# tinganchen/AlignQ

Measured on AMD Instinct MI355X. Metric: images/sec (train step, CDF+ADMM) ResNet-20 8-bit, higher is better.
Workload: dtype f32; 1 GPU; resnet20 CIFAR-shape 3x32x32, 8W/8A CDF+ADMM full train step (cdf_alignment_admm/resnet-20-cifar-10), batch 128/GPU, HIP-graph replay, batch-norm folded into the site kernels, channels-last tensors, all Conv2d_Q convolutions on alignq_conv*_nhwc (exact-product bf16 MFMA); global_batch=128, parallelism=dp1

## Files before the change

### alignq_amd/csrc/conv_kernels.hip

```cpp
#include <hip/hip_runtime.h>
#include <stdint.h>
#include <stdlib.h>

#include "../../include/alignq.h"
#include "site_internal.h"
#include "store_forms.h"
#include "wgrad_reduce_body.h"

namespace {

using namespace alignq_wgr;

typedef __bf16 bf16x8 __attribute__((ext_vector_type(8)));
typedef __bf16 bf16x4 __attribute__((ext_vector_type(4)));
typedef float f32x4 __attribute__((ext_vector_type(4)));
typedef short s16x4 __attribute__((ext_vector_type(4)));

#ifdef ALIGNQ_STAMPS
__device__ unsigned long long g_conv_stamps[64];
__device__ unsigned long long g_conv_blk[2][4096];
#define STAMP(on, i)                                                          \
  do {                                                                        \
    if ((on) && threadIdx.x == 0) g_conv_stamps[i] = wall_clock64();          \
  } while (0)
#define BSTAMP(which)                                                                          \
  do {                                                                                         \
    if (threadIdx.x == 0 && blockIdx.x < 4096) g_conv_blk[which][blockIdx.x] = wall_clock64(); \
  } while (0)
#else
#define STAMP(on, i) do { } while (0)
#define BSTAMP(which) do { } while (0)
#endif

__device__ __forceinline__ s16x4 tr_read(const __bf16* p) {
  return __builtin_amdgcn_ds_read_tr16_b64_v4i16((__attribute__((address_space(3))) s16x4*)(p));
}
__device__ __forceinline__ bf16x8 join8(s16x4 a, s16x4 b) {
  typedef short s16x8 __attribute__((ext_vector_type(8)));
  s16x8 v = {a[0], a[1], a[2], a[3], b[0], b[1], b[2], b[3]};
  return __builtin_bit_cast(bf16x8, v);
}


template <int xb>
__device__ __forceinline__ f32x4 fetch_act4(const float* __restrict__ x, int64_t off) {
  if constexpr (xb == 0) return *reinterpret_cast<const f32x4*>(x + off);
  if constexpr (xb == 2) {
    const s16x4 b = *reinterpret_cast<const s16x4*>(reinterpret_cast<const short*>(x) + off);
    return (f32x4){(float)b[0], (float)b[1], (float)b[2], (float)b[3]};
  }
  const char4 b = *reinterpret_cast<const char4*>(reinterpret_cast<const signed char*>(x) + off);
  return (f32x4){(float)b.x, (float)b.y, (float)b.z, (float)b.w};
}

struct BnLazy {
  const float* z;
  const float* ab;
  const float* save;
  const float* ktot;
  const float* part = nullptr;
  int n_tiles = 0, tile_f = 0;
  double inv_n = 1.0;
  float* dgamma = nullptr;
  float* dbeta = nullptr;
};

template <int C>
__device__ __forceinline__ void bn_totals_lds(const BnLazy& t, float* __restrict__ kt, bool publish) {
  static_assert(256 % C == 0, "thread -> (channel, group)");
  __shared__ double red[256][2];
  constexpr int G = 256 / C;
  const int tid = threadIdx.x;
  const int cp = C < t.tile_f ? C : t.tile_f;
  const int cyc = C / cp, cnt = t.n_tiles / cyc;
  const int c = tid % C, grp = tid / C;
  const int e = c % cp, t_first = c / cp;
  double s0 = 0, s1 = 0;
  constexpr int U = 16;
  for (int i0 = grp; i0 < cnt; i0 += G * U) {
    float2 v[U];
#pragma unroll
    for (int u = 0; u < U; u++) {
      const int i = i0 + u * G;
      const int ic = i < cnt ? i : cnt - 1;
      v[u] = *reinterpret_cast<const float2*>(t.part + ((int64_t)(ic * cyc + t_first) * cp + e) * 2);
    }
#pragma unroll
    for (int u = 0; u < U; u++) {
      if (i0 + u * G < cnt) { s0 += v[u].x; s1 += v[u].y; }
    }
  }
  red[tid][0] = s0;
  red[tid][1] = s1;
  __syncthreads();
  if (tid < C) {
    double t0 = 0, t1 = 0;
#pragma unroll
    for (int g = 0; g < G; g++) { t0 += red[g * C + tid][0]; t1 += red[g * C + tid][1]; }
    kt[tid] = (float)(t0 * t.inv_n);
    kt[C + tid] = (float)(t1 * t.inv_n);
    if (publish) {
      if (t.dbeta) t.dbeta[tid] = (float)t0;
      if (t.dgamma) t.dgamma[tid] = (float)t1;
    }
  }
  __syncthreads();
}

__device__ __forceinline__ float4 bn_lazy4(const float4& g, const float4& z, const float4& a, const float4& m, const float4& is,
                                           const float4& k0, const float4& k1) {
  float4 o;
  o.x = a.x * (g.x - k0.x - (z.x - m.x) * is.x * k1.x);
  o.y = a.y * (g.y - k0.y - (z.y - m.y) * is.y * k1.y);
  o.z = a.z * (g.z - k0.z - (z.z - m.z) * is.z * k1.z);
  o.w = a.w * (g.w - k0.w - (z.w - m.w) * is.w * k1.w);
  return o;
}

template <int C> constexpr int conv_cp() { return C == 16 ? 16 : (C == 32 ? 48 : C + 8); }
template <int C, int WD, int PT>
struct ConvLds {
  static constexpr int kBf16 = 3 * ((PT / WD) + 2) * (WD + 2) * conv_cp<C>();
};

template <int C, int WD, int PT, bool DGRAD, int XB = 0, bool IMG = false>
__device__ __forceinline__ void conv3x3_body(const float* __restrict__ x, const float* __restrict__ w,
                                             float* __restrict__ y, int H, int total_rows, float nlev, __bf16* lds,
                                             int block, const float* __restrict__ add,
                                             float* __restrict__ bn_part = nullptr, int n_wg = 0,
                                             BnLazy lazy = BnLazy{nullptr, nullptr, nullptr, nullptr}, float xlev = 1.0f) {
  static_assert(XB == 0 || !DGRAD, "the data gradient reads fp32 dy");
  constexpr int xb = XB;
  constexpr int TR = PT / WD;
  constexpr int NS = (9 * C + 31) / 32;
  constexpr int NCG = C / 16;
  constexpr int NPP = 4 / NCG;
  constexpr int NG = PT / 16;
  constexpr int LW = WD + 2;
  constexpr int CP = conv_cp<C>();
  constexpr int LROWS = TR + 2;
  constexpr int ARR = LROWS * LW * CP;
  static_assert(3 * ARR == ConvLds<C, WD, PT>::kBf16, "LDS size");
  __bf16* Xhi = lds;
  __bf16* Xmi = lds + ARR;
  __bf16* Xlo = lds + 2 * ARR;

  const int tid = threadIdx.x, lane = tid & 63, wv = tid >> 6;
  const int row0 = block * TR;
  const int img_lo = (row0 / H) * H, img_hi = img_lo + H;
  [[maybe_unused]] constexpr int SB = DGRAD ? 8 : 0;
  STAMP(block == 0, SB + 0);
  const int cog = wv % NCG, pp = wv / NCG;
  const int m = lane & 15, q = lane >> 4;
  bf16x8 ab[NS];
  {
    constexpr int C4 = C / 4;
    constexpr int N4 = LROWS * LW * C4;
    constexpr int NIT = (N4 + 255) / 256;
    float4 v[NIT];
#pragma unroll
    for (int it = 0; it < NIT; it++) {
      const int i = tid + 256 * it;
      const int c4 = i % C4, col = (i / C4) % LW, lr = i / (C4 * LW);
      const int grow = row0 + lr - 1;
      const bool ok = i < N4 && col >= 1 && col <= WD && grow >= img_lo && grow < img_hi && grow < total_rows;
      const int64_t off = ok ? ((int64_t)grow * WD + (col - 1)) * C + 4 * c4 : 0;
      const f32x4 ld = fetch_act4<XB>(x, off);
      v[it] = ok ? make_float4(ld[0], ld[1], ld[2], ld[3]) : make_float4(0.f, 0.f, 0.f, 0.f);
    }
    STAMP(block == 0, SB + 1);
    if (DGRAD && lazy.z) {
      float4 zz[NIT];
#pragma unroll
      for (int it = 0; it < NIT; it++) {
        const int i = tid + 256 * it;
        const int c4 = i % C4, col = (i / C4) % LW, lr = i / (C4 * LW);
        const int grow = row0 + lr - 1;
        const bool ok = i < N4 && col >= 1 && col <= WD && grow >= img_lo && grow < img_hi && grow < total_rows;
        zz[it] = *reinterpret_cast<const float4*>(lazy.z + (ok ? ((int64_t)grow * WD + (col - 1)) * C + 4 * c4 : 0));
      }
      const int c4t = tid % C4;
      const float4 a4 = *reinterpret_cast<const float4*>(lazy.ab + 4 * c4t);
      const float4 m4 = *reinterpret_cast<const float4*>(lazy.save + 4 * c4t);
      const float4 i4 = *reinterpret_cast<const float4*>(lazy.save + C + 4 * c4t);
      float4 k0, k1;
      if (lazy.part) {
        __shared__ __attribute__((aligned(16))) float kt[2 * C];
        bn_totals_lds<C>(lazy, kt, block == 0);
        k0 = *reinterpret_cast<const float4*>(kt + 4 * c4t);
        k1 = *reinterpret_cast<const float4*>(kt + C + 4 * c4t);
      } else {
        k0 = *reinterpret_cast<const float4*>(lazy.ktot + 4 * c4t);
        k1 = *reinterpret_cast<const float4*>(lazy.ktot + C + 4 * c4t);
      }
#pragma unroll
      for (int it = 0; it < NIT; it++) {
        const int i = tid + 256 * it;
        const int col = (i / C4) % LW, lr = i / (C4 * LW);
        const int grow = row0 + lr - 1;
        const bool ok = i < N4 && col >= 1 && col <= WD && grow >= img_lo && grow < img_hi && grow < total_rows;
        if (ok) v[it] = bn_lazy4(v[it], zz[it], a4, m4, i4, k0, k1);
      }
    }
#pragma unroll
    for (int it = 0; it < NIT; it++) {
      const int i = tid + 256 * it;
      if (i < N4) {
        const int c4 = i % C4, col = (i / C4) % LW, lr = i / (C4 * LW);
        bf16x4 h4, m4, l4;
        const float vv[4] = {v[it].x, v[it].y, v[it].z, v[it].w};
#pragma unroll
        for (int e = 0; e < 4; e++) {
          const __bf16 hi = (__bf16)vv[e];
          const float r1 = vv[e] - (float)hi;
          const __bf16 mi = (__bf16)r1;
          const float r2 = r1 - (float)mi;
          h4[e] = hi; m4[e] = mi; l4[e] = (__bf16)r2;
        }
        const int o = (lr * LW + col) * CP + 4 * c4;
        *reinterpret_cast<bf16x4*>(Xhi + o) = h4;
        *reinterpret_cast<bf16x4*>(Xmi + o) = m4;
        *reinterpret_cast<bf16x4*>(Xlo + o) = l4;
      }
    }
    STAMP(block == 0, SB + 2);
    if constexpr (IMG) {
      const bf16x8* __restrict__ wi = reinterpret_cast<const bf16x8*>(w) + (cog * NS) * 64 + lane;
#pragma unroll
      for (int s = 0; s < NS; s++) ab[s] = wi[s * 64];
    } else {
#pragma unroll
      for (int s = 0; s < NS; s++) {
        const int k0 = 32 * s + 8 * q;
        const bool live = k0 / C < 9;
        const int tap = live ? k0 / C : 8, c0 = k0 % C;
        float wr[8];
        if (!DGRAD) {
          const float* p = w + ((int64_t)(cog * 16 + m) * 9 + tap) * C + c0;
          const float4 a4 = *reinterpret_cast<const float4*>(p), b4 = *reinterpret_cast<const float4*>(p + 4);
          wr[0] = a4.x; wr[1] = a4.y; wr[2] = a4.z; wr[3] = a4.w; wr[4] = b4.x; wr[5] = b4.y; wr[6] = b4.z; wr[7] = b4.w;
        } else {
#pragma unroll
          for (int j = 0; j < 8; j++) wr[j] = w[((int64_t)(c0 + j) * 9 + (8 - tap)) * C + cog * 16 + m];
        }
#pragma unroll
        for (int j = 0; j < 8; j++) ab[s][j] = (__bf16)rintf((live ? wr[j] : 0.f) * nlev);
      }
    }
    STAMP(block == 0, SB + 3);
  }
  __syncthreads();
  constexpr int GW = NG / NPP;
  static_assert(NG % NPP == 0, "every wave takes the same number of pixel groups");
  int bo[GW];
  f32x4 acc[GW];
#pragma unroll
  for (int gi = 0; gi < GW; gi++) {
// ... 200 lines not shown
#pragma unroll
  for (int s = 0; s <= NS; s++) {
    if (s < NS) {
      const int k0 = 32 * s + 8 * q;
      const bool live = k0 / CIN < KS * KS;
      const int tap = live ? k0 / CIN : KS * KS - 1, c0 = k0 % CIN;
      const int to = (KS == 3 ? ((tap / KS) * LW + (tap % KS)) * CP : 0) + c0;
#pragma unroll
      for (int gi = 0; gi < GW; gi++) {
        const int o = bo[gi] + to;
        bh[s & 1][gi] = *reinterpret_cast<const bf16x8*>(Xhi + o);
        bm[s & 1][gi] = *reinterpret_cast<const bf16x8*>(Xmi + o);
        bl[s & 1][gi] = *reinterpret_cast<const bf16x8*>(Xlo + o);
        if ((KS * KS * CIN) % 32 != 0 && !live) {
#pragma unroll
          for (int j = 0; j < 8; j++) { bh[s & 1][gi][j] = (__bf16)0.f; bm[s & 1][gi][j] = (__bf16)0.f; bl[s & 1][gi][j] = (__bf16)0.f; }
        }
      }
    }
    __builtin_amdgcn_sched_barrier(0);
    if (s > 0) {
      const int u = s - 1;
#pragma unroll
      for (int gi = 0; gi < GW; gi++) {
        f32x4 a = acc[gi];
        a = __builtin_amdgcn_mfma_f32_16x16x32_bf16(ab[u], bl[u & 1][gi], a, 0, 0, 0);
        a = __builtin_amdgcn_mfma_f32_16x16x32_bf16(ab[u], bm[u & 1][gi], a, 0, 0, 0);
        acc[gi] = __builtin_amdgcn_mfma_f32_16x16x32_bf16(ab[u], bh[u & 1][gi], a, 0, 0, 0);
      }
    }
  }
  float bs[4] = {0.f, 0.f, 0.f, 0.f}, bq[4] = {0.f, 0.f, 0.f, 0.f};
#pragma unroll
  for (int gi = 0; gi < GW; gi++) {
    const int p = (pp + gi * NPP) * 16 + (lane & 15);
    const int r = p / WDO, c = p % WDO;
    const int grow = row0 + r;
    if (grow < total_rows) {
      const float4 v = make_float4(acc[gi][0] / nlev, acc[gi][1] / nlev, acc[gi][2] / nlev, acc[gi][3] / nlev);
      alignq_store::st16<alignq_store::kConvOut>(y + ((int64_t)grow * WDO + c) * COUT + cog * 16 + 4 * q, v);
      bs[0] += v.x; bs[1] += v.y; bs[2] += v.z; bs[3] += v.w;
      bq[0] += v.x * v.x; bq[1] += v.y * v.y; bq[2] += v.z * v.z; bq[3] += v.w * v.w;
    }
  }
  if (bn_part) {
    float* red = reinterpret_cast<float*>(lds);
#define ROW_SHR_ADD(V, CTRL) V += __builtin_bit_cast(float, __builtin_amdgcn_update_dpp(0, __builtin_bit_cast(int, V), CTRL, 0xf, 0xf, false))
#pragma unroll
    for (int e = 0; e < 4; e++) {
      ROW_SHR_ADD(bs[e], 0x111); ROW_SHR_ADD(bs[e], 0x112); ROW_SHR_ADD(bs[e], 0x114); ROW_SHR_ADD(bs[e], 0x118);
      ROW_SHR_ADD(bq[e], 0x111); ROW_SHR_ADD(bq[e], 0x112); ROW_SHR_ADD(bq[e], 0x114); ROW_SHR_ADD(bq[e], 0x118);
    }
#undef ROW_SHR_ADD
    __syncthreads();
    if ((lane & 15) == 15) {
#pragma unroll
      for (int e = 0; e < 4; e++) {
        red[(wv * 16 + 4 * q + e) * 2] = bs[e];
        red[(wv * 16 + 4 * q + e) * 2 + 1] = bq[e];
      }
    }
    __syncthreads();
    if (tid < COUT) {
      const int cg = tid / 16, cl = tid % 16;
      float s0 = 0.f, s1 = 0.f;
#pragma unroll
      for (int ppi = 0; ppi < NPP; ppi++) {
        s0 += red[((ppi * NCG + cg) * 16 + cl) * 2];
        s1 += red[((ppi * NCG + cg) * 16 + cl) * 2 + 1];
      }
      bn_part[((int64_t)tid * n_wg + block) * 2] = s0;
      bn_part[((int64_t)tid * n_wg + block) * 2 + 1] = s1;
    }
  }
}

template <int CIN, int COUT, int WDI, int KS, int S, int PT, bool IMG = false>
__global__ __launch_bounds__(256) void convgen_fwd_kernel(const float* __restrict__ x, const float* __restrict__ w,
                                                          float* __restrict__ y, int H, int total_rows, float nlev,
                                                          float* __restrict__ bn_part) {
  __shared__ __attribute__((aligned(16))) __bf16 lds[3 * ConvGen<CIN, COUT, WDI, KS, S, PT>::ARR];
  convgen_fwd_body<CIN, COUT, WDI, KS, S, PT, IMG>(x, w, y, H, total_rows, nlev, bn_part, lds, blockIdx.x, gridDim.x);
}

template <int CIN, int COUT, int WDI, int PT3, int PT1, bool IMG = false>
__global__ __launch_bounds__(256) void transition_fwd_kernel(const float* __restrict__ x, const float* __restrict__ w3,
                                                             const float* __restrict__ w1, float* __restrict__ y3,
                                                             float* __restrict__ y1, int H, int total_rows, float nlev,
                                                             float* __restrict__ part3, float* __restrict__ part1, int n3) {
  constexpr int A3 = ConvGen<CIN, COUT, WDI, 3, 2, PT3>::ARR, A1 = ConvGen<CIN, COUT, WDI, 1, 2, PT1>::ARR;
  __shared__ __attribute__((aligned(16))) __bf16 lds[3 * (A3 > A1 ? A3 : A1)];
  if ((int)blockIdx.x < n3)
    convgen_fwd_body<CIN, COUT, WDI, 3, 2, PT3, IMG>(x, w3, y3, H, total_rows, nlev, part3, lds, blockIdx.x, n3);
  else
    convgen_fwd_body<CIN, COUT, WDI, 1, 2, PT1, IMG>(x, w1, y1, H, total_rows, nlev, part1, lds, blockIdx.x - n3,
                                                     (int)gridDim.x - n3);
}

template <int CIN, int COUT, int WDI, int KS, int PT, bool WITH1, bool IMG = false>
__device__ __forceinline__ void dgrad_s2_body(const float* __restrict__ dy, const float* __restrict__ w,
                                              float* __restrict__ dx, int H, int total_rows, float nlev,
                                              const float* __restrict__ add, BnLazy lazy, __bf16* lds, int block,
                                              const float* __restrict__ dy1 = nullptr, const float* __restrict__ w1 = nullptr,
                                              BnLazy lazy1 = BnLazy{nullptr, nullptr, nullptr, nullptr}) {
  static_assert(!WITH1 || KS == 3, "the second source is the 1x1 shortcut of a 3x3 transition");
  constexpr int P = KS == 3 ? 1 : 0;
  constexpr int WDO = WDI / 2, TR = PT / WDI;
  constexpr int DROWS = TR / 2 + P, DCOLS = WDO + P;
  constexpr int CP = COUT + 8;
  constexpr int NPIX3 = DROWS * DCOLS + 1;
  constexpr int NPIX1 = WITH1 ? (TR / 2) * WDO : 0;
  constexpr int NPIX = NPIX3 + NPIX1;
  constexpr int ARR = NPIX * CP;
  constexpr int NT = KS * KS + (WITH1 ? 1 : 0);
  constexpr int NS = (NT * COUT + 31) / 32;
  constexpr int NCG = CIN / 16, NPP = 4 / NCG, NG = PT / 16;
  __bf16* Xhi = lds;
  __bf16* Xmi = lds + ARR;
  __bf16* Xlo = lds + 2 * ARR;
  const int tid = threadIdx.x, lane = tid & 63, wv = tid >> 6;
  const int row0 = block * TR;
  const int Ho = H / 2;
  const int orow0 = (row0 / H) * Ho + (row0 % H) / 2;
  const int oimg_hi = (row0 / H + 1) * Ho;
  {
    constexpr int C4 = COUT / 4;
    constexpr int N4 = NPIX3 * C4;
    constexpr int NIT = (N4 + 255) / 256;
    constexpr int M4 = NPIX1 * C4;
    constexpr int NI1 = WITH1 ? (M4 + 255) / 256 : 1;
    float4 v[NIT], zz[NIT], v1[NI1], z1[NI1];
#pragma unroll
    for (int it = 0; it < NIT; it++) {
      const int i = tid + 256 * it;
      const int c4 = i % C4, pix = i / C4;
      const int lr = pix / DCOLS, col = pix % DCOLS;
      const int grow = orow0 + lr;
      const bool ok = i < N4 && pix < DROWS * DCOLS && col < WDO && grow < oimg_hi;
      const int64_t off = ok ? ((int64_t)grow * WDO + col) * COUT + 4 * c4 : 0;
      v[it] = *reinterpret_cast<const float4*>(dy + off);
      if (lazy.z) zz[it] = *reinterpret_cast<const float4*>(lazy.z + off);
      if (!ok) v[it] = make_float4(0.f, 0.f, 0.f, 0.f);
    }
    if constexpr (WITH1) {
#pragma unroll
      for (int it = 0; it < NI1; it++) {
        const int i = tid + 256 * it;
        const int64_t off = i < M4 ? ((int64_t)orow0 * WDO) * COUT + 4 * (int64_t)i : 0;
        v1[it] = *reinterpret_cast<const float4*>(dy1 + off);
        if (lazy1.z) z1[it] = *reinterpret_cast<const float4*>(lazy1.z + off);
      }
    }
    const int c4t = tid % C4;
    if (lazy.z) {
      const float4 a4 = *reinterpret_cast<const float4*>(lazy.ab + 4 * c4t);
      const float4 m4 = *reinterpret_cast<const float4*>(lazy.save + 4 * c4t);
      const float4 i4 = *reinterpret_cast<const float4*>(lazy.save + COUT + 4 * c4t);
      float4 k0, k1;
      if (lazy.part) {
        __shared__ __attribute__((aligned(16))) float kt[2 * COUT];
        bn_totals_lds<COUT>(lazy, kt, block == 0);
        k0 = *reinterpret_cast<const float4*>(kt + 4 * c4t);
        k1 = *reinterpret_cast<const float4*>(kt + COUT + 4 * c4t);
      } else {
        k0 = *reinterpret_cast<const float4*>(lazy.ktot + 4 * c4t);
        k1 = *reinterpret_cast<const float4*>(lazy.ktot + COUT + 4 * c4t);
      }
#pragma unroll
      for (int it = 0; it < NIT; it++) {
        const int i = tid + 256 * it;
        const int pix = i / C4;
        const int lr = pix / DCOLS, col = pix % DCOLS;
        const bool ok = i < N4 && pix < DROWS * DCOLS && col < WDO && orow0 + lr < oimg_hi;
        if (ok) v[it] = bn_lazy4(v[it], zz[it], a4, m4, i4, k0, k1);
      }
    }
    if constexpr (WITH1) {
      if (lazy1.z) {
        const float4 a4 = *reinterpret_cast<const float4*>(lazy1.ab + 4 * c4t);
        const float4 m4 = *reinterpret_cast<const float4*>(lazy1.save + 4 * c4t);
        const float4 i4 = *reinterpret_cast<const float4*>(lazy1.save + COUT + 4 * c4t);
        float4 k0, k1;
        if (lazy1.part) {
          __shared__ __attribute__((aligned(16))) float kt1[2 * COUT];
          bn_totals_lds<COUT>(lazy1, kt1, block == 0);
          k0 = *reinterpret_cast<const float4*>(kt1 + 4 * c4t);
          k1 = *reinterpret_cast<const float4*>(kt1 + COUT + 4 * c4t);
        } else {
          k0 = *reinterpret_cast<const float4*>(lazy1.ktot + 4 * c4t);
          k1 = *reinterpret_cast<const float4*>(lazy1.ktot + COUT + 4 * c4t);
        }
#pragma unroll
        for (int it = 0; it < NI1; it++) {
          if (tid + 256 * it < M4) v1[it] = bn_lazy4(v1[it], z1[it], a4, m4, i4, k0, k1);
        }
      }
    }
#pragma unroll
    for (int it = 0; it < NIT + (WITH1 ? NI1 : 0); it++) {
      const bool second = it >= NIT;
      const int i = tid + 256 * (second ? it - NIT : it);
      if (i < (second ? M4 : N4)) {
        const int c4 = i % C4, pix = (second ? NPIX3 : 0) + i / C4;
        bf16x4 h4, m4, l4;
        const float4 src = second ? v1[second ? it - NIT : 0] : v[second ? 0 : it];
        const float vv[4] = {src.x, src.y, src.z, src.w};
#pragma unroll
        for (int e = 0; e < 4; e++) {
          const __bf16 hi = (__bf16)vv[e];
          const float r1 = vv[e] - (float)hi;
          const __bf16 mi = (__bf16)r1;
          h4[e] = hi; m4[e] = mi; l4[e] = (__bf16)(r1 - (float)mi);
        }
        const int o = pix * CP + 4 * c4;
        *reinterpret_cast<bf16x4*>(Xhi + o) = h4;
        *reinterpret_cast<bf16x4*>(Xmi + o) = m4;
        *reinterpret_cast<bf16x4*>(Xlo + o) = l4;
      }
    }
  }
  const int cig = wv % NCG, pp = wv / NCG;
  const int m = lane & 15, q = lane >> 4;
  bf16x8 ab[NS];
  if constexpr (IMG) {
    static_assert((KS * KS * COUT) % 32 == 0 && COUT % 32 == 0, "whole k steps per filter");
    constexpr int NS3 = KS * KS * COUT / 32;
    const bf16x8* __restrict__ wi = reinterpret_cast<const bf16x8*>(w) + (cig * NS3) * 64 + lane;
#pragma unroll
    for (int s = 0; s < NS3; s++) ab[s] = wi[s * 64];
    if constexpr (WITH1) {
      const bf16x8* __restrict__ wj = reinterpret_cast<const bf16x8*>(w1) + (cig * (NS - NS3)) * 64 + lane;
#pragma unroll
      for (int s = NS3; s < NS; s++) ab[s] = wj[(s - NS3) * 64];
    }
  } else {
#pragma unroll
    for (int s = 0; s < NS; s++) {
      const int k0 = 32 * s + 8 * q;
      const int tap = k0 / COUT, c0 = k0 % COUT;
#pragma unroll
      for (int j = 0; j < 8; j++) {
        float v = 0.f;
        if (tap < KS * KS) v = w[((int64_t)(c0 + j) * (KS * KS) + tap) * CIN + cig * 16 + m];
        else if (WITH1 && tap == KS * KS) v = w1[(int64_t)(c0 + j) * CIN + cig * 16 + m];
        ab[s][j] = (__bf16)rintf(v * nlev);
      }
    }
  }
  __syncthreads();
  for (int g = pp; g < NG; g += NPP) {
    const int p = g * 16 + (lane & 15);
    const int r = p / WDI, c = p % WDI;
    f32x4 acc = {0.f, 0.f, 0.f, 0.f};
#pragma unroll
    for (int s = 0; s < NS; s++) {
      const int k0 = 32 * s + 8 * q;
      const int tap = k0 / COUT, c0 = k0 % COUT;
      int pix = DROWS * DCOLS;
      if (tap < KS * KS) {
        const int ky = tap / KS, kx = tap % KS;
        const int a = r + P - ky, b = c + P - kx;
        if (a >= 0 && b >= 0 && !(a & 1) && !(b & 1)) pix = (a >> 1) * DCOLS + (b >> 1);
      } else if (WITH1 && tap == KS * KS) {
        if (!(r & 1) && !(c & 1)) pix = NPIX3 + (r >> 1) * WDO + (c >> 1);
      }
      const int o = pix * CP + c0;
      const bf16x8 bh = *reinterpret_cast<const bf16x8*>(Xhi + o);
      const bf16x8 bm = *reinterpret_cast<const bf16x8*>(Xmi + o);
      const bf16x8 bl = *reinterpret_cast<const bf16x8*>(Xlo + o);
      acc = __builtin_amdgcn_mfma_f32_16x16x32_bf16(ab[s], bl, acc, 0, 0, 0);
      acc = __builtin_amdgcn_mfma_f32_16x16x32_bf16(ab[s], bm, acc, 0, 0, 0);
      acc = __builtin_amdgcn_mfma_f32_16x16x32_bf16(ab[s], bh, acc, 0, 0, 0);
    }
    const int grow = row0 + r;
    if (grow < total_rows) {
      const int64_t o = ((int64_t)grow * WDI + c) * CIN + cig * 16 + 4 * q;
      float4 out = make_float4(acc[0] / nlev, acc[1] / nlev, acc[2] / nlev, acc[3] / nlev);
      if (add) {
        const float4 a4 = *reinterpret_cast<const float4*>(add + o);
        out.x += a4.x; out.y += a4.y; out.z += a4.z; out.w += a4.w;
      }
      alignq_store::st16<alignq_store::kConvOut>(dx + o, out);
    }
  }
}

template <int CIN, int COUT, int WDI, int KS, int PT, bool WITH1>
struct DgradS2Lds {
  static constexpr int P = KS == 3 ? 1 : 0, TR = PT / WDI;
  static constexpr int kBf16 = 3 * (((TR / 2 + P) * (WDI / 2 + P) + 1) + (WITH1 ? (TR / 2) * (WDI / 2) : 0)) * (COUT + 8);
};

template <int CIN, int COUT, int WDI, int KS, int PT, bool IMG = false>
__global__ __launch_bounds__(256) void dgrad_s2_kernel(const float* __restrict__ dy, const float* __restrict__ w,
                                                       float* __restrict__ dx, int H, int total_rows, float nlev,
                                                       const float* __restrict__ add, BnLazy lazy) {
  __shared__ __attribute__((aligned(16))) __bf16 lds[DgradS2Lds<CIN, COUT, WDI, KS, PT, false>::kBf16];
  dgrad_s2_body<CIN, COUT, WDI, KS, PT, false, IMG>(dy, w, dx, H, total_rows, nlev, add, lazy, lds, blockIdx.x);
}

template <int CIN, int COUT, int WDI, int KS, int PT>
int launch_dgrad_s2(const float* dy, const float* w, float* dx, int B, int H, float nlev, const float* add, BnLazy lazy,
                    hipStream_t st, bool img = false) {
  constexpr int TR = PT / WDI;
  static_assert(TR % 2 == 0, "even number of input rows per tile");
  if (H % TR) return ALIGNQ_EUNSUPPORTED;
  const int total_rows = B * H;
  if (img)
    hipLaunchKernelGGL((dgrad_s2_kernel<CIN, COUT, WDI, KS, PT, true>), total_rows / TR, 256, 0, st, dy, w, dx, H, total_rows, nlev,
                       add, lazy);
  else
    hipLaunchKernelGGL((dgrad_s2_kernel<CIN, COUT, WDI, KS, PT>), total_rows / TR, 256, 0, st, dy, w, dx, H, total_rows, nlev,
                       add, lazy);
  hipError_t e = hipGetLastError();
  return e == hipSuccess ? 0 : (int)e;
}

constexpr int kStemPT = 128;
__device__ __forceinline__ void stem_stage(const float* __restrict__ x, int H, int row0, __bf16* Chi, __bf16* Cmi, __bf16* Clo) {
  const int tid = threadIdx.x;
  const int pix = tid >> 1, half = tid & 1;
  const int r = pix / 32, c = pix % 32;
  const int grow = row0 + r;
  const int ih = grow % H;
  float v[16];
#pragma unroll
  for (int j = 0; j < 16; j++) {
    const int k = 16 * half + j;
    const int tap = k / 3, ci = k % 3;
    const int ky = tap / 3, kx = tap % 3;
    const int yy = ih + ky - 1, xx = c + kx - 1;
    const bool ok = k < 27 && yy >= 0 && yy < H && xx >= 0 && xx < 32;
    v[j] = x[ok ? ((int64_t)(grow + ky - 1) * 32 + xx) * 3 + ci : 0];
    if (!ok) v[j] = 0.f;
  }
  bf16x8 h[2], m[2], l[2];
#pragma unroll
  for (int j = 0; j < 16; j++) {
    const __bf16 hi = (__bf16)v[j];
    const float r1 = v[j] - (float)hi;
    const __bf16 mi = (__bf16)r1;
    h[j >> 3][j & 7] = hi; m[j >> 3][j & 7] = mi; l[j >> 3][j & 7] = (__bf16)(r1 - (float)mi);
  }
  const int o = pix * 32 + 16 * half;
  *reinterpret_cast<bf16x8*>(Chi + o) = h[0]; *reinterpret_cast<bf16x8*>(Chi + o + 8) = h[1];
  *reinterpret_cast<bf16x8*>(Cmi + o) = m[0]; *reinterpret_cast<bf16x8*>(Cmi + o + 8) = m[1];
  *reinterpret_cast<bf16x8*>(Clo + o) = l[0]; *reinterpret_cast<bf16x8*>(Clo + o + 8) = l[1];
// ... 334 lines not shown
      }
    }
    __syncthreads();
    STAMP(st_on && tile - t_begin < 16, 18 + 2 * (tile - t_begin));
    nxt = tile + 1;
    if (nxt < t_end) {
      const int row0_ = nxt * TR;
      const int img_lo_ = (row0_ / H) * (H * S), img_hi_ = img_lo_ + H * S;
#pragma unroll
      for (int it = 0; it < NIX; it++) {
        const int i = tid + 256 * it;
        const int c4 = i % C4, col = (i / C4) % LW, lr = i / (C4 * LW);
        const int grow = KS == 3 ? row0_ * S - 1 + lr : (row0_ + lr) * S;
        const int gcol = KS == 3 ? col - 1 : col * S;
        const bool ok = i < N4 && gcol >= 0 && gcol < WDI && grow >= img_lo_ && grow < img_hi_;
        const int64_t off = ok ? ((int64_t)grow * WDI + gcol) * CIN + bj * CB + 4 * c4 : 0;
        rx[it] = fetch_act4<XB>(x, off);
        if (!ok) rx[it] = (f32x4){0.f, 0.f, 0.f, 0.f};
      }
#pragma unroll
      for (int it = 0; it < NID; it++) {
        const int i = tid + 256 * it;
        const int64_t off = i < M4 ? ((int64_t)row0_ * WDO + i / C4) * COUT + bi * CB + 4 * (i % C4) : 0;
        rd[it] = *reinterpret_cast<const f32x4*>(dy + off);
        if (lazy.z) rz[it] = *reinterpret_cast<const f32x4*>(lazy.z + off);
      }
    }
    for (int s = (CB == 16 ? wv : 0); s < NSTEP; s += (CB == 16 ? 4 : 1)) {
      const int p0 = 32 * s + 8 * g;
      const int r = p0 / WDO, c0 = p0 % WDO;
      bf16x8 a[3];
#pragma unroll
      for (int t = 0; t < 3; t++) {
        const __bf16* pa = Di[t] + (p0 + q) * CB + cob * 16 + pcol;
        a[t] = join8(tr_read(pa), tr_read(pa + 4 * CB));
      }
#pragma unroll
      for (int tap = 0; tap < NT; tap++) {
        const int ky = tap / KS, kx = tap % KS;
        bf16x8 b[3];
#pragma unroll
        for (int t = 0; t < 3; t++) {
          const __bf16* pb = Xi[t] + (KS == 3 ? ((r * S + ky) * LW + ((c0 + q) * S + kx)) : (r * LW + c0 + q)) * CB +
                             cib * 16 + pcol;
          b[t] = join8(tr_read(pb), tr_read(pb + 4 * (KS == 3 ? S : 1) * CB));
        }
        f32x4 v = acc[tap];
        v = __builtin_amdgcn_mfma_f32_16x16x32_bf16(a[1], b[1], v, 0, 0, 0);
        if (xb == 0) v = __builtin_amdgcn_mfma_f32_16x16x32_bf16(a[0], b[2], v, 0, 0, 0);
        v = __builtin_amdgcn_mfma_f32_16x16x32_bf16(a[2], b[0], v, 0, 0, 0);
        v = __builtin_amdgcn_mfma_f32_16x16x32_bf16(a[0], b[1], v, 0, 0, 0);
        v = __builtin_amdgcn_mfma_f32_16x16x32_bf16(a[1], b[0], v, 0, 0, 0);
        v = __builtin_amdgcn_mfma_f32_16x16x32_bf16(a[0], b[0], v, 0, 0, 0);
        acc[tap] = v;
      }
    }
    STAMP(st_on && tile - t_begin < 16, 19 + 2 * (tile - t_begin));
  }
  STAMP(st_on, 50);
  float* slab = slabs + (int64_t)bx * (NT * CIN * COUT);
  if (xb != 0) {
    const float inv = 1.0f / xlev;
#pragma unroll
    for (int t = 0; t < NT; t++) acc[t] = acc[t] * inv;
  }
  if (CB == 16) {
    float* red = lds_f;
    __syncthreads();
    if (wv > 0) {
#pragma unroll
      for (int t = 0; t < NT; t++)
#pragma unroll
        for (int e = 0; e < 4; e++) red[(((wv - 1) * NT + t) * 4 + e) * 64 + lane] = acc[t][e];
    }
    __syncthreads();
    if (wv == 0) {
#pragma unroll
      for (int t = 0; t < NT; t++) {
#pragma unroll
        for (int e = 0; e < 4; e++) {
          float v = acc[t][e];
#pragma unroll
          for (int w2 = 0; w2 < 3; w2++) v += red[((w2 * NT + t) * 4 + e) * 64 + lane];
          alignq_store::st4<alignq_store::kConvWgradSlab, true>(&slab[((int64_t)(bi * CB + 4 * (lane >> 4) + e) * NT + t) * CIN + bj * CB + (lane & 15)], v);
        }
      }
    }
  } else {
#pragma unroll
    for (int t = 0; t < NT; t++)
#pragma unroll
      for (int e = 0; e < 4; e++)
        alignq_store::st4<alignq_store::kConvWgradSlab, true>(&slab[((int64_t)(bi * CB + cob * 16 + 4 * (lane >> 4) + e) * NT + t) * CIN + bj * CB + cib * 16 + (lane & 15)], acc[t][e]);
  }
  STAMP(st_on, 51);
}

template <int C, int WD, int PT, int XB = 0>
__device__ __forceinline__ void wgrad3x3_body(const float* __restrict__ x, const float* __restrict__ dy,
                                              float* __restrict__ slabs, int H, int n_tiles, float* lds_f, int bx, int gx,
                                              int by, BnLazy lazy = BnLazy{nullptr, nullptr, nullptr, nullptr}, float xlev = 1.0f) {
  wgrad_body<C, C, WD, 3, 1, PT, XB>(x, dy, slabs, H, n_tiles, lds_f, bx, gx, by, lazy, xlev);
}

template <int CIN, int COUT, int WDI, int KS, int S, int PT>
__global__ __launch_bounds__(256) void wgradgen_kernel(const float* __restrict__ x, const float* __restrict__ dy,
                                                       float* __restrict__ slabs, int H, int n_tiles, BnLazy lazy) {
  __shared__ __attribute__((aligned(16))) float lds[WgradGeo<CIN, COUT, WDI, KS, S, PT>::kFloats];
  wgrad_body<CIN, COUT, WDI, KS, S, PT>(x, dy, slabs, H, n_tiles, lds, blockIdx.x, gridDim.x, blockIdx.y, lazy);
}

template <int C, int WD, int PT, int XB>
__global__ __launch_bounds__(256) void wgrad3x3_nhwc_kernel(const float* __restrict__ x, const float* __restrict__ dy,
                                                            float* __restrict__ slabs, int H, int n_tiles, float xlev) {
  __shared__ __attribute__((aligned(16))) float lds[WgradLds<C, WD, PT>::kFloats];
  wgrad3x3_body<C, WD, PT, XB>(x, dy, slabs, H, n_tiles, lds, blockIdx.x, gridDim.x, blockIdx.y,
                               BnLazy{nullptr, nullptr, nullptr, nullptr}, xlev);
}

template <int C, int WD, int PTD, int PTW, int XB, bool IMG = false>
__global__ __launch_bounds__(256) __attribute__((amdgpu_waves_per_eu(C == 16 ? 3 : 2, C == 16 ? 3 : 8)))
void conv3x3_bwd_kernel(const float* __restrict__ x, const float* __restrict__ dy,
                                                          const float* __restrict__ w, float* __restrict__ dx,
                                                          float* __restrict__ slabs, int H, int total_rows, float nlev,
                                                          int n_tiles_w, int splits, int nblk2,
                                                          const float* __restrict__ add, BnLazy lazy, float xlev, int dg_R,
                                                          RedFill fill, int n_dg) {
  constexpr int kBytesD = ConvLds<C, WD, PTD>::kBf16 * 2, kBytesW = WgradLds<C, WD, PTW>::kFloats * 4;
  static_assert(kBytesD >= 4096 || kBytesW >= 4096, "the filler role's 4 KB");
  __shared__ __attribute__((aligned(16))) unsigned char lds[kBytesD > kBytesW ? kBytesD : kBytesW];
  const int n_wg = splits * nblk2;
  BSTAMP(0);
  if ((int)blockIdx.x < n_wg) {
    wgrad3x3_body<C, WD, PTW, XB>(x, dy, slabs, H, n_tiles_w, reinterpret_cast<float*>(lds), blockIdx.x % splits, splits,
                                  blockIdx.x / splits, lazy, xlev);
  } else if ((int)blockIdx.x >= n_wg + n_dg) {
    const int fb = blockIdx.x - n_wg - n_dg;
    int it = 0;
    while (it + 1 < kFill && fb >= fill.blk0[it + 1]) it++;
    wgrad_reduce_body<256>(fill.slabs[it], fill.n_slabs[it], fill.n_elem[it], fill.dw[it], fb - fill.blk0[it],
                           reinterpret_cast<float*>(lds));
  } else {
    int m = blockIdx.x - n_wg;
    if (dg_R > 0) {
      const int i = (m / (8 * dg_R)) * 8 + (m & 7), r = (m >> 3) % dg_R;
      m = dg_R * i + r;
    }
    conv3x3_body<C, WD, PTD, true, 0, IMG>(dy, w, dx, H, total_rows, nlev, reinterpret_cast<__bf16*>(lds), m, add, nullptr, 0, lazy);
  }
  BSTAMP(1);
}

template <int CIN, int COUT, int WDI, int PTW3, int PTW1, int PTD, bool IMG = false>
__global__ __launch_bounds__(256) void transition_bwd_kernel(const float* __restrict__ x, const float* __restrict__ dy3,
                                                             const float* __restrict__ dy1, const float* __restrict__ w3,
                                                             const float* __restrict__ w1, float* __restrict__ dx,
                                                             float* __restrict__ slabs3, float* __restrict__ slabs1, int Ho,
                                                             int n_tiles3, int n_tiles1, int splits3, int splits1, int n_d,
                                                             float nlev, const float* __restrict__ add, BnLazy lazy3,
                                                             BnLazy lazy1, int dg_R) {
  using G3 = WgradGeo<CIN, COUT, WDI, 3, 2, PTW3>;
  using G1 = WgradGeo<CIN, COUT, WDI, 1, 2, PTW1>;
  constexpr int NBY = (COUT / G3::CB) * (CIN / G3::CB);
  static_assert(G3::CB == G1::CB, "same channel blocking");
  constexpr int kD = DgradS2Lds<CIN, COUT, WDI, 3, PTD, true>::kBf16 * 2;
  constexpr int kW = G3::kBytes > G1::kBytes ? G3::kBytes : G1::kBytes;
  __shared__ __attribute__((aligned(16))) unsigned char lds[kD > kW ? kD : kW];
  const int n_w3 = splits3 * NBY;
  const int b = blockIdx.x;
  if (b < n_d) {
    int m = b;
    if (dg_R > 0) {
      const int i = (m / (8 * dg_R)) * 8 + (m & 7), r = (m >> 3) % dg_R;
      m = dg_R * i + r;
    }
    dgrad_s2_body<CIN, COUT, WDI, 3, PTD, true, IMG>(dy3, w3, dx, 2 * Ho, 0x7fffffff, nlev, add, lazy3,
                                                     reinterpret_cast<__bf16*>(lds), m, dy1, w1, lazy1);
  } else if (b < n_d + n_w3) {
    const int c = b - n_d;
    wgrad_body<CIN, COUT, WDI, 3, 2, PTW3>(x, dy3, slabs3, Ho, n_tiles3, reinterpret_cast<float*>(lds), c % splits3, splits3,
                                           c / splits3, lazy3);
  } else {
    const int c = b - n_d - n_w3;
    wgrad_body<CIN, COUT, WDI, 1, 2, PTW1>(x, dy1, slabs1, Ho, n_tiles1, reinterpret_cast<float*>(lds), c % splits1, splits1,
                                           c / splits1, lazy1);
  }
}

__global__ __launch_bounds__(1024) void wgrad_reduce_kernel(const float* __restrict__ slabs, int n_slabs, int n_elem,
                                                            float* __restrict__ dw) {
  __shared__ __attribute__((aligned(16))) float part[4096];
  wgrad_reduce_body(slabs, n_slabs, n_elem, dw, blockIdx.x, part);
}

constexpr int kWgMulti = 32;
struct WgChunk {
  const float* slabs[kWgMulti];
  float* dw[kWgMulti];
  int n_slabs[kWgMulti];
  int n_elem[kWgMulti];
  int blk0[kWgMulti + 1];
};
__global__ __launch_bounds__(1024) void wgrad_reduce_multi_kernel(WgChunk c, int cnt) {
  __shared__ __attribute__((aligned(16))) float part[4096];
  int t = 0;
  while (t + 1 < cnt && (int)blockIdx.x >= c.blk0[t + 1]) t++;
  wgrad_reduce_body(c.slabs[t], c.n_slabs[t], c.n_elem[t], c.dw[t], (int)blockIdx.x - c.blk0[t], part);
}

template <int C, int WD, int PT>
int launch_wgrad(const float* x, const float* dy, float* dw, float* ws, int B, int H, int* n_slabs_out, hipStream_t st,
                 int xb = 0, float xlev = 1.0f) {
  constexpr int TR = PT / WD;
  if (H % TR) return ALIGNQ_EUNSUPPORTED;
  const int n_tiles = B * H / TR;
  constexpr int NB = (C >= 32 ? C / 32 : 1);
  int splits = 256 / (NB * NB);
  if (splits > n_tiles) splits = n_tiles;
  if (xb == 2) hipLaunchKernelGGL((wgrad3x3_nhwc_kernel<C, WD, PT, 2>), dim3(splits, NB * NB), 256, 0, st, x, dy, ws, H, n_tiles, xlev);
  else if (xb == 1) hipLaunchKernelGGL((wgrad3x3_nhwc_kernel<C, WD, PT, 1>), dim3(splits, NB * NB), 256, 0, st, x, dy, ws, H, n_tiles, xlev);
  else hipLaunchKernelGGL((wgrad3x3_nhwc_kernel<C, WD, PT, 0>), dim3(splits, NB * NB), 256, 0, st, x, dy, ws, H, n_tiles, xlev);
  hipError_t e = hipGetLastError();
  if (e != hipSuccess) return (int)e;
  if (n_slabs_out) { *n_slabs_out = splits; return 0; }
  const int n_elem = 9 * C * C;
  hipLaunchKernelGGL(wgrad_reduce_kernel, wgrad_reduce_blocks(splits, n_elem), 1024, 0, st, ws, splits, n_elem, dw);
  e = hipGetLastError();
  return e == hipSuccess ? 0 : (int)e;
}

template <int C, int WD, int PTD, int PTW>
int launch_bwd(const float* x, const float* dy, const float* w, float* dx, float* ws, int B, int H, float nlev,
               int* n_slabs_out, const float* add, BnLazy lazy, hipStream_t st, int xb, float xlev, const RedFill& fill,
               bool img) {
  constexpr int TRD = PTD / WD, TRW = PTW / WD;
  if (H % TRD || H % TRW) return ALIGNQ_EUNSUPPORTED;
  const int total_rows = B * H;
  const int n_tiles_w = total_rows / TRW;
  constexpr int NB = (C >= 32 ? C / 32 : 1);
  int splits = 256 / (NB * NB);
  if (splits > n_tiles_w) splits = n_tiles_w;
  const int n_d = total_rows / TRD;
  const int grid = splits * NB * NB + n_d + fill.blk0[kFill];
  const int per = (n_tiles_w + splits - 1) / splits;
  int dg_R = 0;
  if ((per * TRW) % TRD == 0 && (splits * NB * NB) % 8 == 0 && splits % 8 == 0) {
    const int R = per * TRW / TRD;
    if (R >= 1 && R * splits == n_d) dg_R = R;
  }
#define LBW(XBV, IM) hipLaunchKernelGGL((conv3x3_bwd_kernel<C, WD, PTD, PTW, XBV, IM>), grid, 256, 0, st, x, dy, w, dx, ws, H, total_rows, nlev, n_tiles_w, splits, NB * NB, add, lazy, xlev, dg_R, fill, n_d)
  if (img) {
    if (xb == 2) LBW(2, true); else if (xb == 1) LBW(1, true); else LBW(0, true);
  } else if (xb == 2) LBW(2, false); else if (xb == 1) LBW(1, false); else LBW(0, false);
#undef LBW
  hipError_t e = hipGetLastError();
  if (e != hipSuccess) return (int)e;
  *n_slabs_out = splits;
  return 0;
}

template <int CIN, int COUT, int WDI, int KS, int S, int PT>
int launch_wgradgen(const float* x, const float* dy, float* dw, float* ws, int B, int H, int* n_slabs_out, BnLazy lazy,
                    hipStream_t st) {
  using G = WgradGeo<CIN, COUT, WDI, KS, S, PT>;
  if (H % G::TR) return ALIGNQ_EUNSUPPORTED;
  const int n_tiles = B * H / G::TR;
  constexpr int NBY = (COUT / G::CB) * (CIN / G::CB);
  int splits = 256 / NBY;
  if (splits > n_tiles) splits = n_tiles;
  hipLaunchKernelGGL((wgradgen_kernel<CIN, COUT, WDI, KS, S, PT>), dim3(splits, NBY), 256, 0, st, x, dy, ws, H, n_tiles, lazy);
  hipError_t e = hipGetLastError();
  if (e != hipSuccess) return (int)e;
  if (n_slabs_out) { *n_slabs_out = splits; return 0; }
  const int n_elem = G::NT * CIN * COUT;
  hipLaunchKernelGGL(wgrad_reduce_kernel, wgrad_reduce_blocks(splits, n_elem), 1024, 0, st, ws, splits, n_elem, dw);
  e = hipGetLastError();
  return e == hipSuccess ? 0 : (int)e;
}

template <int CIN, int COUT, int WDI, int PT3, int PT1>
int launch_transition_fwd(const float* x, const float* w3, const float* w1, float* y3, float* y1, int B, int H, float nlev,
                          float* part3, float* part1, hipStream_t st, bool img) {
  constexpr int TR3 = ConvGen<CIN, COUT, WDI, 3, 2, PT3>::TR, TR1 = ConvGen<CIN, COUT, WDI, 1, 2, PT1>::TR;
  if (H % TR3 || H % TR1) return ALIGNQ_EUNSUPPORTED;
  const int total_rows = B * H, n3 = total_rows / TR3, n1 = total_rows / TR1;
  if (img)
    hipLaunchKernelGGL((transition_fwd_kernel<CIN, COUT, WDI, PT3, PT1, true>), n3 + n1, 256, 0, st, x, w3, w1, y3, y1, H,
                       total_rows, nlev, part3, part1, n3);
  else
    hipLaunchKernelGGL((transition_fwd_kernel<CIN, COUT, WDI, PT3, PT1>), n3 + n1, 256, 0, st, x, w3, w1, y3, y1, H, total_rows,
                       nlev, part3, part1, n3);
  hipError_t e = hipGetLastError();
  return e == hipSuccess ? 0 : (int)e;
}

template <int CIN, int COUT, int WDI, int PTW3, int PTW1, int PTD>
int launch_transition_bwd(const float* x, const float* dy3, const float* dy1, const float* w3, const float* w1, float* dx,
                          float* ws3, float* ws1, int B, int Ho, float nlev, int* ns3, int* ns1, const float* add,
                          BnLazy lazy3, BnLazy lazy1, hipStream_t st, bool img) {
  using G3 = WgradGeo<CIN, COUT, WDI, 3, 2, PTW3>;
  using G1 = WgradGeo<CIN, COUT, WDI, 1, 2, PTW1>;
  constexpr int TRD = PTD / WDI;
  if (Ho % G3::TR || Ho % G1::TR || (2 * Ho) % TRD) return ALIGNQ_EUNSUPPORTED;
  const int n_tiles3 = B * Ho / G3::TR, n_tiles1 = B * Ho / G1::TR;
  constexpr int NBY = (COUT / G3::CB) * (CIN / G3::CB);
  int splits3 = 256 / NBY, splits1 = 256 / NBY;
  if (splits3 > n_tiles3) splits3 = n_tiles3;
// ... 440 lines not shown
```

Baseline: 142,200 images/sec.

## Merge dual BN-total reductions into one interleaved pass, add occupancy hint

```diff
diff --git a/alignq_amd/csrc/conv_kernels.hip b/alignq_amd/csrc/conv_kernels.hip
--- a/alignq_amd/csrc/conv_kernels.hip
+++ b/alignq_amd/csrc/conv_kernels.hip
@@ -65,44 +65,107 @@
   float* dbeta = nullptr;
 };
 
+template <int C> constexpr int bn_totals_u() { return C == 32 ? 32 : 16; }
+template <int C, int Uv = bn_totals_u<C>()>
+struct BnTotalsGeo {
+  static constexpr int G = 256 / C, U = Uv, R = 8;
+  int cnt, nfull, cyc, cp, e, t_first, grp;
+  unsigned off0, stride;
+  __device__ __forceinline__ explicit BnTotalsGeo(const BnLazy& t) {
+    static_assert(256 % C == 0, "thread -> (channel, group)");
+    const int tid = threadIdx.x;
+    cp = C < t.tile_f ? C : t.tile_f;
+    cyc = C / cp; cnt = t.n_tiles / cyc;
+    nfull = cnt / G;
+    const int c = tid % C;
+    grp = tid / C; e = c % cp; t_first = c / cp;
+    off0 = (unsigned)((grp * cyc + t_first) * cp + e) * 2u;
+    stride = (unsigned)(G * cyc * cp) * 2u;
+  }
+  __device__ __forceinline__ void request(const BnLazy& t, int j, float2 (&v)[U]) const {
+#pragma unroll
+    for (int u = 0; u < U; u++) {
+      const float* row = t.part + (size_t)((unsigned)(j + u) * stride);
+      v[u] = *reinterpret_cast<const float2*>(row + off0);
+    }
+  }
+  __device__ __forceinline__ void add(const float2 (&v)[U], double& s0, double& s1) const {
+#pragma unroll
+    for (int u = 0; u < U; u++) { s0 += v[u].x; s1 += v[u].y; }
+  }
+  __device__ __forceinline__ void rest(const BnLazy& t, int j, float2 (&v)[U], double& s0, double& s1) const {
+    for (; j + U <= nfull; j += U) {
+      request(t, j, v);
+      add(v, s0, s1);
+    }
+    for (; j * G < cnt; j += R) {
+      float2 r[R];
+#pragma unroll
+      for (int u = 0; u < R; u++) {
+        const int i = grp + (j + u) * G;
+        const int ic = i < cnt ? i : cnt - 1;
+        r[u] = *reinterpret_cast<const float2*>(t.part + (unsigned)((ic * cyc + t_first) * cp + e) * 2u);
+      }
+#pragma unroll
+      for (int u = 0; u < R; u++) {
+        if (grp + (j + u) * G < cnt) { s0 += r[u].x; s1 += r[u].y; }
+      }
+    }
+  }
+};
 template <int C>
+__device__ __forceinline__ void bn_totals_finish(const BnLazy& t, const double (*red)[2], int c, float* __restrict__ kt, bool publish) {
+  constexpr int G = 256 / C;
+  double t0 = 0, t1 = 0;
+#pragma unroll
+  for (int g = 0; g < G; g++) { t0 += red[g * C + c][0]; t1 += red[g * C + c][1]; }
+  kt[c] = (float)(t0 * t.inv_n);
+  kt[C + c] = (float)(t1 * t.inv_n);
+  if (publish) {
+    if (t.dbeta) t.dbeta[c] = (float)t0;
+    if (t.dgamma) t.dgamma[c] = (float)t1;
+  }
+}
+template <int C, int Uv = bn_totals_u<C>()>
 __device__ __forceinline__ void bn_totals_lds(const BnLazy& t, float* __restrict__ kt, bool publish) {
-  static_assert(256 % C == 0, "thread -> (channel, group)");
+  using Geo = BnTotalsGeo<C, Uv>;
   __shared__ double red[256][2];
-  constexpr int G = 256 / C;
   const int tid = threadIdx.x;
-  const int cp = C < t.tile_f ? C : t.tile_f;
-  const int cyc = C / cp, cnt = t.n_tiles / cyc;
-  const int c = tid % C, grp = tid / C;
-  const int e = c % cp, t_first = c / cp;
+  const Geo geo(t);
   double s0 = 0, s1 = 0;
-  constexpr int U = 16;
-  for (int i0 = grp; i0 < cnt; i0 += G * U) {
-    float2 v[U];
-#pragma unroll
-    for (int u = 0; u < U; u++) {
-      const int i = i0 + u * G;
-      const int ic = i < cnt ? i : cnt - 1;
-      v[u] = *reinterpret_cast<const float2*>(t.part + ((int64_t)(ic * cyc + t_first) * cp + e) * 2);
-    }
-#pragma unroll
-    for (int u = 0; u < U; u++) {
-      if (i0 + u * G < cnt) { s0 += v[u].x; s1 += v[u].y; }
-    }
-  }
+  float2 v[Geo::U];
+  geo.rest(t, 0, v, s0, s1);
   red[tid][0] = s0;
   red[tid][1] = s1;
   __syncthreads();
+  if (tid < C) bn_totals_finish<C>(t, red, tid, kt, publish);
+  __syncthreads();
+}
+template <int C>
+__device__ __forceinline__ void bn_totals_lds2(const BnLazy& ta, const BnLazy& tb, bool on0, bool on1, float* __restrict__ kta,
+                                               float* __restrict__ ktb, bool publish, double (*red)[2]) {
+  using Geo = BnTotalsGeo<C, 16>;
+  static_assert(2 * C <= 256, "one finishing thread per record and channel");
+  const int tid = threadIdx.x;
+  const Geo ga(on0 ? ta : tb), gb(on1 ? tb : ta);
+  double a0 = 0, a1 = 0, b0 = 0, b1 = 0;
+  float2 va[Geo::U], vb[Geo::U];
+  const bool ra = on0 && Geo::U <= ga.nfull, rb = on1 && Geo::U <= gb.nfull;
+  if (ra) ga.request(ta, 0, va);
+  if (rb) gb.request(tb, 0, vb);
+  if (ra) ga.add(va, a0, a1);
+  if (on0) ga.rest(ta, ra ? Geo::U : 0, va, a0, a1);
+  if (rb) gb.add(vb, b0, b1);
+  if (on1) gb.rest(tb, rb ? Geo::U : 0, vb, b0, b1);
+  red[tid][0] = a0;
+  red[tid][1] = a1;
+  red[256 + tid][0] = b0;
+  red[256 + tid][1] = b1;
+  __syncthreads();
   if (tid < C) {
-    double t0 = 0, t1 = 0;
-#pragma unroll
-    for (int g = 0; g < G; g++) { t0 += red[g * C + tid][0]; t1 += red[g * C + tid][1]; }
-    kt[tid] = (float)(t0 * t.inv_n);
-    kt[C + tid] = (float)(t1 * t.inv_n);
-    if (publish) {
-      if (t.dbeta) t.dbeta[tid] = (float)t0;
-      if (t.dgamma) t.dgamma[tid] = (float)t1;
-    }
+    if (on0) bn_totals_finish<C>(ta, red, tid, kta, publish);
+  } else if (tid < 2 * C) {
+    if (on1) bn_totals_finish<C>(tb, red + 256, tid - C, ktb, publish);
   }
   __syncthreads();
 }
@@ -609,20 +672,47 @@
       }
     }
     const int c4t = tid % C4;
-    if (lazy.z) {
-      const float4 a4 = *reinterpret_cast<const float4*>(lazy.ab + 4 * c4t);
-      const float4 m4 = *reinterpret_cast<const float4*>(lazy.save + 4 * c4t);
-      const float4 i4 = *reinterpret_cast<const float4*>(lazy.save + COUT + 4 * c4t);
-      float4 k0, k1;
-      if (lazy.part) {
-        __shared__ __attribute__((aligned(16))) float kt[2 * COUT];
-        bn_totals_lds<COUT>(lazy, kt, block == 0);
+    const bool lz0 = lazy.z != nullptr, lz1 = WITH1 && lazy1.z != nullptr;
+    const bool pt0 = lz0 && lazy.part, pt1 = lz1 && lazy1.part;
+    const float4 zero4 = make_float4(0.f, 0.f, 0.f, 0.f);
+    float4 a4 = zero4, m4 = zero4, i4 = zero4, k0 = zero4, k1 = zero4;
+    float4 a41 = zero4, m41 = zero4, i41 = zero4, k01 = zero4, k11 = zero4;
+    if (lz0) {
+      a4 = *reinterpret_cast<const float4*>(lazy.ab + 4 * c4t);
+      m4 = *reinterpret_cast<const float4*>(lazy.save + 4 * c4t);
+      i4 = *reinterpret_cast<const float4*>(lazy.save + COUT + 4 * c4t);
+      if (!pt0) {
+        k0 = *reinterpret_cast<const float4*>(lazy.ktot + 4 * c4t);
+        k1 = *reinterpret_cast<const float4*>(lazy.ktot + COUT + 4 * c4t);
+      }
+    }
+    if (lz1) {
+      a41 = *reinterpret_cast<const float4*>(lazy1.ab + 4 * c4t);
+      m41 = *reinterpret_cast<const float4*>(lazy1.save + 4 * c4t);
+      i41 = *reinterpret_cast<const float4*>(lazy1.save + COUT + 4 * c4t);
+      if (!pt1) {
+        k01 = *reinterpret_cast<const float4*>(lazy1.ktot + 4 * c4t);
+        k11 = *reinterpret_cast<const float4*>(lazy1.ktot + COUT + 4 * c4t);
+      }
+    }
+    if (pt0 || pt1) {
+      __shared__ __attribute__((aligned(16))) float kt[(WITH1 ? 4 : 2) * COUT];
+      if constexpr (WITH1) {
+        static_assert(3 * ARR * sizeof(__bf16) >= 2 * 256 * 2 * sizeof(double), "the two records' group sums lie in the tile image");
+        bn_totals_lds2<COUT>(lazy, lazy1, pt0, pt1, kt, kt + 2 * COUT, block == 0, reinterpret_cast<double(*)[2]>(lds));
+      } else {
+        bn_totals_lds<COUT, 16>(lazy, kt, block == 0);
+      }
+      if (pt0) {
         k0 = *reinterpret_cast<const float4*>(kt + 4 * c4t);
         k1 = *reinterpret_cast<const float4*>(kt + COUT + 4 * c4t);
-      } else {
-        k0 = *reinterpret_cast<const float4*>(lazy.ktot + 4 * c4t);
-        k1 = *reinterpret_cast<const float4*>(lazy.ktot + COUT + 4 * c4t);
-      }
+      }
+      if (WITH1 && pt1) {
+        k01 = *reinterpret_cast<const float4*>(kt + 2 * COUT + 4 * c4t);
+        k11 = *reinterpret_cast<const float4*>(kt + 3 * COUT + 4 * c4t);
+      }
+    }
+    if (lz0) {
 #pragma unroll
       for (int it = 0; it < NIT; it++) {
         const int i = tid + 256 * it;
@@ -633,23 +723,10 @@
       }
     }
     if constexpr (WITH1) {
-      if (lazy1.z) {
-        const float4 a4 = *reinterpret_cast<const float4*>(lazy1.ab + 4 * c4t);
-        const float4 m4 = *reinterpret_cast<const float4*>(lazy1.save + 4 * c4t);
-        const float4 i4 = *reinterpret_cast<const float4*>(lazy1.save + COUT + 4 * c4t);
-        float4 k0, k1;
-        if (lazy1.part) {
-          __shared__ __attribute__((aligned(16))) float kt1[2 * COUT];
-          bn_totals_lds<COUT>(lazy1, kt1, block == 0);
-          k0 = *reinterpret_cast<const float4*>(kt1 + 4 * c4t);
-          k1 = *reinterpret_cast<const float4*>(kt1 + COUT + 4 * c4t);
-        } else {
-          k0 = *reinterpret_cast<const float4*>(lazy1.ktot + 4 * c4t);
-          k1 = *reinterpret_cast<const float4*>(lazy1.ktot + COUT + 4 * c4t);
-        }
+      if (lz1) {
 #pragma unroll
         for (int it = 0; it < NI1; it++) {
-          if (tid + 256 * it < M4) v1[it] = bn_lazy4(v1[it], z1[it], a4, m4, i4, k0, k1);
+          if (tid + 256 * it < M4) v1[it] = bn_lazy4(v1[it], z1[it], a41, m41, i41, k01, k11);
         }
       }
     }
@@ -1290,7 +1367,7 @@
 }
 
 template <int CIN, int COUT, int WDI, int PTW3, int PTW1, int PTD, bool IMG = false>
-__global__ __launch_bounds__(256) void transition_bwd_kernel(const float* __restrict__ x, const float* __restrict__ dy3,
+__global__ __launch_bounds__(256) __attribute__((amdgpu_waves_per_eu(2))) void transition_bwd_kernel(const float* __restrict__ x, const float* __restrict__ dy3,
                                                              const float* __restrict__ dy1, const float* __restrict__ w3,
                                                              const float* __restrict__ w1, float* __restrict__ dx,
                                                              float* __restrict__ slabs3, float* __restrict__ slabs1, int Ho,
```

After: 142,400 images/sec, median of 5. No clear change (+0.2%).
